# przemo199/ray-tracer-challenge-rs

Measured on AMD Instinct MI355X. Metric: Mray/s (primary+secondary) and ms/frame at 1920x1080, higher is better.
Workload: dtype f32; 1 GPU; three_sphere_scene@1920x1080,depth=5,f32; scene=three_sphere_scene, width=1920, height=1080, max_depth=5, out=real, parallelism=framesx1, rays_per_frame=4147200, stream=side, mode=frames

## Files before the change

### include/rtc_scene.h

```cpp
#ifndef RTC_SCENE_H
#define RTC_SCENE_H

#include "rtc.h"

#ifdef __cplusplus
extern "C" {
#endif

typedef struct rt_scene rt_scene;

typedef struct rt_scene_view {
    const rt_shape_desc* shapes;
    uint32_t n_shapes;
    const rt_material_desc* materials;
    uint32_t n_materials;
    const rt_pattern_desc* patterns;
    uint32_t n_patterns;
    const rt_light_desc* lights;
    uint32_t n_lights;
    rt_camera_desc camera;
    uint32_t duplicate_shapes;
} rt_scene_view;

int rt_scene_load_yaml(const char* path, rt_scene** out);
// ... 9 lines not shown
    const uint32_t* triangles;
    uint32_t n_triangles;
    uint32_t ignored_lines;
} rt_mesh_view;

int rt_mesh_load_obj(const char* path, rt_mesh** out);
int rt_mesh_load_obj_text(const char* text, rt_mesh** out);
int rt_mesh_view_get(const rt_mesh* mesh, rt_mesh_view* view);
void rt_mesh_free(rt_mesh* mesh);

int rt_mesh_triangles(const rt_mesh* mesh, const double* transform, int bake, int32_t material, rt_shape_desc* out);

#define RT_OBJ_NORMALS 1u
#define RT_NO_NORMAL 0xFFFFFFFFu
int rt_mesh_load_obj_ex(const char* path, const char* text, uint32_t flags, rt_mesh** out);

typedef struct rt_mesh_normals_view {
    const double* normals;
    uint32_t n_normals;
    uint32_t n_smooth;
    const uint32_t* triangle_normals;
} rt_mesh_normals_view;
int rt_mesh_normals_get(const rt_mesh* mesh, rt_mesh_normals_view* view);

int rt_mesh_smooth_normals(const rt_mesh* mesh, const double* transform, int bake, rt_smooth_desc* out,
                           uint32_t list, uint32_t* n_out);

#define RT_OBJ_TEXCOORDS 4u
#define RT_NO_TEXCOORD 0xFFFFFFFFu
typedef struct rt_mesh_texcoords_view {
    const double* texcoords;
    uint32_t n_texcoords;
    uint32_t n_textured;
    const uint32_t* triangle_texcoords;
} rt_mesh_texcoords_view;
int rt_mesh_texcoords_get(const rt_mesh* mesh, rt_mesh_texcoords_view* view);
int rt_mesh_uvs(const rt_mesh* mesh, rt_uv_desc* out, uint32_t list, uint32_t* n_out);

int rt_camera_make(uint32_t width, uint32_t height, double field_of_view,
                   const double from[3], const double to[3], const double up[3],
                   rt_camera_desc* out);

int rt_camera_resize(rt_camera_desc* camera, uint32_t width, uint32_t height);

int rt_camera_set_transform(rt_camera_desc* camera, const double transform[16]);

int rt_camera_bound_rect(const rt_camera_desc* camera, const float bound[4], uint32_t rect[4]);

int rt_camera_shadow_rect(const rt_camera_desc* camera, const float plane[4], const float light[3],
                          const float bound[4], uint32_t rect[4]);

int rt_camera_shadow_near(const rt_camera_desc* camera, const float plane[4], const float light[3], uint32_t span[4]);

int rt_matrix_inverse(const double m[16], double out[16]);

int rt_image_write(const char* path, const uint8_t* rgb, uint32_t width, uint32_t height);

enum {
    RT_IMAGE_AUTO = 0,
    RT_IMAGE_PNG = 1,
    RT_IMAGE_PPM = 2,
    RT_IMAGE_PPM_BINARY = 3
};
int rt_image_write_format(const char* path, const uint8_t* rgb, uint32_t width, uint32_t height, int format);

int rt_canvas_quantize(const double* rgb, uint64_t n_channels, uint8_t* out);

#ifdef __cplusplus
}
#endif

#endif
```

### ray-tracer-challenge-rs_amd/csrc/primary_rect.hpp

```cpp
#pragma once

#include <cmath>
#include <cstdint>

#include "rtc_internal.hpp"

namespace rtc {

enum ConicExtent { kConicFull, kConicOff, kConicRect };
struct ConicForm {
    double ad[3][3];
};
inline bool conic_form(const double m[3][3], const double oc[3], double R, ConicForm& f) {
    double g[3][3] = {}, q[3] = {}, oo = 0.0;
    for (int i = 0; i < 3; ++i)
        for (int j = 0; j < 3; ++j)
            for (int k = 0; k < 3; ++k) g[i][j] += m[k][i] * m[k][j];
    for (int i = 0; i < 3; ++i) oo += oc[i] * oc[i];
    for (int i = 0; i < 3; ++i)
        for (int k = 0; k < 3; ++k) q[i] += m[k][i] * oc[k];
    const double k = oo - R * R;
    if (!(k > 1e-6 * oo) || !std::isfinite(k)) return false;
    double c[3][3];
    for (int i = 0; i < 3; ++i)
// ... 175 lines not shown
        qa += S * S * f1 * f1, qb += S * S * f0 * f1, qc += S * S * f0 * f0;
        const double disc = qb * qb - qa * qc;
        if (!std::isfinite(disc) || !(disc > 0.0) || qa == 0.0) return false;
        const double root = std::sqrt(disc);
        const double u1 = (-qb - root) / qa, u2 = (-qb + root) / qa;
        if (qa < 0.0) {
            lo = u2, hi = u1;
            return f0 + f1 * 0.5 * (lo + hi) > 0.0;
        }
        if (f1 > 0.0) lo = u2, hi = HUGE_VAL;
        else if (f1 < 0.0) lo = -HUGE_VAL, hi = u1;
        else return false;
        return true;
    };
    auto axis = [&](bool rows, uint32_t n_pix, uint32_t n_other, uint32_t& lo, uint32_t& hi) {
        double lo_a, hi_a, lo_b, hi_b;
        const double e0 = -1.0, e1 = (double)n_other;
        if (rows ? !line_span(e0, 0.0, 0.0, 1.0, lo_a, hi_a) || !line_span(e1, 0.0, 0.0, 1.0, lo_b, hi_b)
                 : !line_span(0.0, e0, 1.0, 0.0, lo_a, hi_a) || !line_span(0.0, e1, 1.0, 0.0, lo_b, hi_b))
            return;
        const double a = std::fmax(std::fmax(lo_a, lo_b), -1.0), b = std::fmin(std::fmin(hi_a, hi_b), (double)n_pix);
        if (!(a <= b)) return;
        const double ai = std::ceil(a), bi = std::floor(b);
        if (!(ai <= bi)) return;
        if (rows ? !near_at(e0, ai) || !near_at(e1, ai) || !near_at(e0, bi) || !near_at(e1, bi)
                 : !near_at(ai, e0) || !near_at(ai, e1) || !near_at(bi, e0) || !near_at(bi, e1))
            return;
        if (ai + 1.0 > bi - 1.0) return;
        lo = (uint32_t)(ai + 1.0);
        hi = (uint32_t)(bi - 1.0);
    };
    axis(false, width, height, span[0], span[2]);
    axis(true, height, width, span[1], span[3]);
}

inline bool shadow_self_clear(const CameraRec<float>& cam, const float n[3], float h, const float light[3]) {
    double nn = 0.0, no = 0.0, nl = 0.0, omax = 0.0, lmax = 0.0;
    for (int i = 0; i < 3; ++i) {
        nn += (double)n[i] * n[i];
        no += (double)n[i] * cam.origin[i];
        nl += (double)n[i] * light[i];
        omax = std::fmax(omax, std::fabs((double)cam.origin[i]));
        lmax = std::fmax(lmax, std::fabs((double)light[i]));
    }
    nn = std::sqrt(nn);
    if (!(nn > 0.0) || !std::isfinite(nn)) return false;
    const double ye = (no - (double)h) / nn, yl = (nl - (double)h) / nn;
    const double scale = 1.0 + omax + lmax + std::fabs((double)h) / nn;
    if (!std::isfinite(ye) || !std::isfinite(yl) || !(ye * yl > 0.0)) return false;
    if (!(std::fabs(ye) > 1e-3 * scale) || !(std::fabs(yl) > 1e-3 * scale)) return false;
    const double over_max = 3e-6 * (1.0 + omax + std::fabs(ye) * nn / 8e-8);
    return over_max <= 1e3 * std::fabs(yl);
}
}
```

### ray-tracer-challenge-rs_amd/csrc/rtc_host.cpp

```cpp
#include <hip/hip_runtime.h>

#include <algorithm>
#include <array>
#include <chrono>
#include <cmath>
#include <cstdlib>
#include <cstring>
#include <limits>
#include <memory>
#include <string>
#include <vector>

#include "../../include/rtc.h"
#include "flop_model.hpp"
#include "host_math.hpp"
#include "debug_knobs.hpp"
#include "launch_terms.hpp"
#include "primary_rect.hpp"
#include "rtc_context.hpp"
#include "rtc_internal.hpp"
#include "shape_identity.hpp"
#include "tri_tree.hpp"
#include "instances.hpp"

// ... 854 lines not shown
        P.spill_blocks = (uint32_t)(ctx->d_spill.capacity() / per_block);
    }
    P.persistent = ls.sched;
    P.flags = flags;
    P.world_lds = ls.world_lds;
    const bool dynamic = ls.pool;
    if (dynamic) {
        const size_t set = (size_t)kTileQueues * kQueueStride;
        P.tile_counter = ctx->d_tile_counter.get() + (ctx->head_set ? set : 0);
        P.next_tile_counter = ctx->d_tile_counter.get() + (ctx->head_set ? 0 : set);
        if (ls.pool && ctx->knobs.tile_order && cam) {
            if ((rc = plan_tile_order<R>(ctx, lens ? ctx->order_lens : ss ? ctx->order_ss : ctx->order, P, cam, depth,
                                         ls.grid, stream, q.lens)))
                return rc;
        }
    }
    if (flags & RT_FLAG_STAMPS) {
        if ((rc = ctx->d_stamps.reserve((size_t)2 * ls.grid))) return rc;
        P.stamps = ctx->d_stamps.get();
        ctx->stamp_count = ls.grid;
        if (ls.pool) {
            const size_t items = (size_t)P.n_tiles << kMaxSplitLog2;
            if ((rc = ctx->d_item_log.reserve(1 + 3 * items))) return rc;
            RT_HIP(hipMemsetAsync(ctx->d_item_log.get(), 0, sizeof(uint64_t), stream));
            P.item_log = ctx->d_item_log.get();
        }
    }
    uint32_t kinds = 0;
    for (int k = 0; k < kNumKinds; ++k)
        if (w.scene.kind_begin[k + 1] > w.scene.kind_begin[k]) kinds |= 1u << k;
    const bool sp = sizeof(R) == 4 && ls.pool && ctx->knobs.kind_variants && (kinds & ~kKindsSp) == 0 && !dup && !ss &&
                    ctx->kernel_build == KernelBuild::plain;
    if (flags & RT_FLAG_FAIL_LAUNCH) return set_error(RT_ERR_HIP, "launch refused (RT_FLAG_FAIL_LAUNCH)");
    if constexpr (sizeof(R) == 4) {
        const size_t ns = ctx->jit.shapes.size();
        const bool small_direct = jf && !ls.pool && cam && !ss && ns <= (size_t)kPrimaryRectSlots &&
                                  (int)ns == w.scene.kind_begin[kNumKinds];
        if (small_direct) launch_terms(ctx->jit.shapes.data(), w.scene.kind_begin, (int)ns, P.cam.origin, P.terms);
        if (small_direct && P.width <= kCullCols * kCullCellW && P.height <= kCullRows * kCullCellH) {
            const uint32_t nc = (P.width + kCullCellW - 1) / kCullCellW, nr = (P.height + kCullCellH - 1) / kCullCellH;
            uint32_t flip_cols[kCullCols + 1] = {}, flip_rows[kCullRows + 1] = {};
            auto outside = [&](const uint32_t r[4], uint32_t b) {
                const bool none = r[0] > r[2] || r[1] > r[3];
                const uint32_t c0 = none ? nc : r[0] / kCullCellW, c1 = none ? nc : r[2] / kCullCellW + 1;
                const uint32_t r0 = none ? nr : r[1] / kCullCellH, r1 = none ? nr : r[3] / kCullCellH + 1;
                flip_cols[0] ^= b, flip_cols[c0] ^= b, flip_cols[c1] ^= b;
                flip_rows[0] ^= b, flip_rows[r0] ^= b, flip_rows[r1] ^= b;
            };
            for (size_t s = 0; s < ns; ++s) {
                uint32_t r[4];
                primary_rect(P.cam, P.width, P.height, ctx->jit.shapes[s].bound, r);
                outside(r, 1u << s);
            }
            const ShadowLayout lay(w.scene.kind_begin, (int)ctx->jit.lights.size());
            if (lay.fits() &&(int)ctx->jit.lights.size() == w.scene.n_lights) {
                for (int p = lay.plane0; p < lay.plane0 + lay.planes; ++p) {
                    const ShapeRec<float>& pl = ctx->jit.shapes[p];
                    const float n[3] = {pl.inv[4], pl.inv[5], pl.inv[6]}, h = -pl.inv[7];
                    uint32_t near[4] = {0, 0, P.width - 1, P.height - 1};
                    for (int l = 0; l < lay.lights; ++l) {
                        const float* lp = ctx->jit.lights[l].position;
                        uint32_t sp[4];
                        shadow_near(P.cam, P.width, P.height, n, h, lp, sp);
                        for (int a = 0; a < 2; ++a) {
                            near[a] = sp[a] > near[a] ? sp[a] : near[a];
                            near[a + 2] = sp[a + 2] < near[a + 2] ? sp[a + 2] : near[a + 2];
                        }
                        for (size_t c = 0; c < ns; ++c) {
                            const int bit = lay.pair_bit(l, p, (int)c);
                            if (bit < 0) continue;
                            if ((int)c == p) {
                                if (shadow_self_clear(P.cam, n, h, lp)) flip_cols[0] ^= 1u << bit;
                                continue;
                            }
                            uint32_t r[4];
                            shadow_rect(P.cam, P.width, P.height, n, h, lp, ctx->jit.shapes[c].bound, r);
                            outside(r, 1u << bit);
                        }
                    }
                    auto blocks = [](uint32_t lo, uint32_t hi, uint32_t cell, uint32_t pixels, uint32_t& b0, uint32_t& b1) {
                        b0 = b1 = 0;
                        if (lo > hi) return;
                        b0 = (lo + cell - 1) / cell;
                        b1 = hi + 1 >= pixels ? (pixels + cell - 1) / cell : (hi + 1) / cell;
                        if (b1 < b0) b1 = b0;
                    };
                    const uint32_t nb = 1u << lay.near_bit(p);
                    uint32_t b0, b1;
                    blocks(near[0], near[2], kCullCellW, P.width, b0, b1);
                    flip_cols[b0] ^= nb, flip_cols[b1] ^= nb;
                    blocks(near[1], near[3], kCullCellH, P.height, b0, b1);
                    flip_rows[b0] ^= nb, flip_rows[b1] ^= nb;
                }
            }
            uint32_t acc = 0;
            for (uint32_t i = 0; i < nc; ++i) P.cull_cols[i] = acc ^= flip_cols[i];
            acc = 0;
            for (uint32_t j = 0; j < nr; ++j) P.cull_rows[j] = acc ^= flip_rows[j];
        }
    }
    if (jf) {
        const ShapeRec<R>* sh = P.scene.shapes;
        const MaterialRec<R>* mt = P.scene.materials;
        const PatternRec<R>* pt = P.scene.patterns;
        const LightRec<R>* lt = P.scene.lights;
        void* args[] = {&P, &sh, &mt, &pt, &lt, &lens_params};
// ... 1715 lines not shown
```

### ray-tracer-challenge-rs_amd/csrc/rtc_kernels.hip

```cpp
#ifndef RTC_INSTANCES
#define RTC_INSTANCES 0
#endif
#ifndef RTC_AREA_LIGHTS
#define RTC_AREA_LIGHTS 0
#endif
#ifndef RTC_TEXTURES
#define RTC_TEXTURES 0
#endif
#if defined(RTC_VARIANT) && !RTC_INSTANCES
#define RTC_POOL_ONLY 1
#endif
#ifndef __HIPCC_RTC__
#include <hip/hip_runtime.h>

#include <cstdint>
#endif

#include "rtc_internal.hpp"

namespace rtc {
#ifdef RTC_VARIANT
namespace RTC_VARIANT {
#endif

// ... 743 lines not shown
            const int32_t e = P.inst_pos[inst[k].pos_begin + (hw - inst[k].world_base)];
            const bool plain = inst[k].expanded != 0;
            h.slot = plain ? (int)((uint32_t)e & 0xFFFFFFu) : e;
            h.kind = plain ? (int)((uint32_t)e >> 24) : (RT_SHAPE_TRIANGLE | ((k + 1) << 8));
            return h;
        }
#endif
        if (hw != __INT_MAX__) {
            const uint32_t ws = (uint32_t)sc.lworld_slot[hw];
            h.slot = (int)(ws & 0xFFFFFFu);
            h.kind = (int)(ws >> 24);
        }
        return h;
    }
};

#ifndef RTC_CUBE_EXIT_PATH
#define RTC_CUBE_EXIT_PATH 1
#endif
template <typename R>
__device__ inline bool jit_cube_holds_light(const ShapeRec<R>& s) {
#if defined(RTC_JIT) && RTC_CUBE_EXIT_PATH
    if constexpr (sizeof(R) == 4) {
        bool any = false;
        for (int i = 0; i < jit::kNumLights; ++i) {
            const V3<R> p = xform_point(s.inv, V3<R>{jit::kLights[i].position[0], jit::kLights[i].position[1],
                                                     jit::kLights[i].position[2]});
            constexpr R kIn = (R)(1 - 1e-4);
            any |= Real<R>::fabs(p.x) < kIn && Real<R>::fabs(p.y) < kIn && Real<R>::fabs(p.z) < kIn;
        }
        return any;
    }
#endif
    (void)s;
    return false;
}

template <typename R>
__device__ inline bool skips_on(const DevScene<R>& sc) {
#ifdef RTC_NO_SKIPS
    (void)sc;
    return false;
#else
#ifdef RTC_JIT
    if constexpr (sizeof(R) == 4) return true;
#endif
    return !sc.no_skips;
#endif
}

#ifndef RTC_PRIMARY_RECTS
#define RTC_PRIMARY_RECTS 1
#endif
struct NoBlock {
    static constexpr bool kOn = false;
    __device__ bool misses(int) const { return false; }
    __device__ float plane_height(int) const { return 0.0f; }
    __device__ float origin_max() const { return 0.0f; }
};
#ifndef RTC_LAUNCH_TERMS
#define RTC_LAUNCH_TERMS 1
#endif
#ifdef RTC_JIT
constexpr int kJitPlane0 = jit::kBegin[RT_SHAPE_PLANE];
constexpr int kJitPlanes = jit::kBegin[RT_SHAPE_PLANE + 1] - kJitPlane0;
#else
constexpr int kJitPlane0 = 0, kJitPlanes = 0;
#endif
struct PixelBlock {
    static constexpr bool kOn = true;
    uint32_t miss;
    __device__ inline bool misses(int slot) const { return (miss >> slot) & 1u; }
    static constexpr int kHead = kJitPlanes <= kPrimaryRectSlots ? (1 + kJitPlanes + 3) / 4 * 4 : 4;
    float head[kHead];
    __device__ inline float plane_height(int plane) const { return head[1 + plane]; }
    __device__ inline float origin_max() const { return head[0]; }
};

template <typename R, typename B = NoBlock>
__device__ inline Hit<R> closest_hit(const DevScene<R>& sc, V3<R> o, V3<R> d, B blk = B{}) {
    Nearest<R> best;
#if defined(RTC_JIT) && !defined(RTC_NO_SKIPS) && RTC_PRIMARY_RECTS
    constexpr bool kRects = B::kOn && sizeof(R) == 4 && jit::kBegin[kNumKinds] <= kPrimaryRectSlots;
    constexpr bool kLazy = kRects && jit::kNumClusters == 0;
#else
    constexpr bool kRects = false, kLazy = false;
#endif
#if defined(RTC_JIT) && RTC_LAUNCH_TERMS
    constexpr bool kTerms = B::kOn && sizeof(R) == 4 && jit::kBegin[kNumKinds] <= kPrimaryRectSlots;
#else
    constexpr bool kTerms = false;
#endif
    R dd0 = (R)0, rdd0 = (R)0;
    V3<R> rd0 = {(R)0, (R)0, (R)0};
    if constexpr (!kLazy) {
        dd0 = dot(d, d);
        rdd0 = recip(dd0);
        rd0 = recip3(d);
    }
    for_all_culled<R, true>(sc, o, d, dd0, [&]<int K>(const ShapeRec<R>& s, int slot) {
        if constexpr (kTerms) jit_fence_dir(d, slot);
        else jit_fence(o, d, slot);
        if constexpr (kRects && K != RT_SHAPE_PLANE)
            if (blk.misses(slot)) return;
        const R dd = kLazy ? dot(d, d) : dd0;
        if (!wave_may_hit<R, K>(s, o, d, dd)) return;
        const int w = kJitRecords && sizeof(R) == 4 ? (s.world_index << 8) | slot : s.world_index;
        if (world_sphere<R, K>(s)) {
            const R rdd = kLazy ? recip(dd) : rdd0;
            sphere_world<R, true>(s, o, d, dd, rdd, [&](R t, bool v) { best.offer(t, v, w); });
            return;
        }
        if (world_cube<R, K>(s)) {
            const V3<R> rd = kLazy ? recip3(d) : rd0;
            cube_world<R, true>(s, o, d, rd, [&](R t, bool v) { best.offer(t, v, w); });
            return;
        }
        V3<R> lo = {(R)0, (R)0, (R)0};
        if constexpr (kTerms && K == RT_SHAPE_PLANE) lo.y = blk.plane_height(slot - kJitPlane0);
        else lo = xform_point(s.inv, o);
        const V3<R> ld = xform_vector(s.inv, d);
        if (K == RT_SHAPE_PLANE && skips_on(sc)) {
            if (!wave_any(!(lo.y * ld.y > (R)0))) return;
        }
        if constexpr (K == RT_SHAPE_CUBE && sizeof(R) == 4) {
            if (jit_cube_holds_light(s) && skips_on(sc) &&
                !wave_any(!(Real<R>::fabs(lo.x) < (R)1 && Real<R>::fabs(lo.y) < (R)1 && Real<R>::fabs(lo.z) < (R)1))) {
                using T = Real<R>;
                auto hi = [](auto org, auto dir) {
                    const bool steep = T::fabs(dir) >= T::kEps;
                    const R r = sel(steep, __builtin_amdgcn_rcpf(dir), T::kMax);
                    return sel(r > (R)0, (R)1 - org, (R)-1 - org) * r;
                };
                const R tmax = T::fmin(T::fmin(T::fmin(T::kMax, hi(lo.x, ld.x)), hi(lo.y, ld.y)), hi(lo.z, ld.z));
                best.offer(tmax, tmax > (R)0, w);
                return;
            }
        }
        entries<R, K, true>(s, lo, ld, [&](R t, bool v) { best.offer(t, v, w); });
    });
    return best.hit(sc);
}

template <typename R>
struct Blocker {
    static constexpr bool kKeys = sizeof(R) == 4 && RTC_VALU_KEYS;
    bool hit = false;
    uint32_t tmin = 0x7F800000u;
    __device__ inline void offer(R t, bool v, R dist) {
        if constexpr (kKeys) {
            const uint32_t b = __float_as_uint((v ? t : -1.0f) + 0.0f);
            tmin = b < tmin ? b : tmin;
        } else {
            hit |= v & (t >= (R)0) & (t < dist);
        }
    }
// ... 2170 lines not shown
```

### ray-tracer-challenge-rs_amd/csrc/scene_loader.cpp

```cpp
#include <cerrno>
#include <cstdlib>
#include <cstring>
#include <fstream>
#include <map>
#include <memory>
#include <sstream>
#include <stdexcept>
#include <string>
#include <vector>

#include "../../include/rtc_scene.h"
#include "host_math.hpp"
#include "primary_rect.hpp"
#include "rtc_internal.hpp"
#include "shape_identity.hpp"

namespace rtc {
namespace {

using hm::M4;

struct Node {
    enum Kind { Bad, Null, Bool, Int, Real, Str, Seq, Map } kind = Bad;
    bool b = false;
    int64_t i = 0;
    std::string s;
    std::vector<Node> seq;
    std::vector<std::pair<std::string, Node>> map;

    const Node& operator[](const std::string& key) const {
        static const Node bad;
        if (kind != Map) return bad;
        const Node* hit = &bad;
        for (const auto& kv : map)
            if (kv.first == key) hit = &kv.second;
        return *hit;
    }
    bool is_bad() const { return kind == Bad; }
};

[[noreturn]] void fail(const std::string& msg) { throw std::runtime_error(msg); }

bool rust_parse_f64(const std::string& v, double& out) {
    std::string t = v;
    size_t p = 0;
    if (p < t.size() && (t[p] == '+' || t[p] == '-')) ++p;
    std::string rest = t.substr(p);
    std::string low;
    for (char c : rest) low += (char)std::tolower((unsigned char)c);
    if (low == "inf" || low == "infinity" || low == "nan") {
        double r = (low == "nan") ? NAN : INFINITY;
        out = (t[0] == '-') ? -r : r;
        return true;
    }
    size_t q = p, digits = 0;
    while (q < t.size() && std::isdigit((unsigned char)t[q])) ++q, ++digits;
    if (q < t.size() && t[q] == '.') {
        ++q;
        while (q < t.size() && std::isdigit((unsigned char)t[q])) ++q, ++digits;
    }
    if (digits == 0) return false;
    if (q < t.size() && (t[q] == 'e' || t[q] == 'E')) {
        ++q;
        if (q < t.size() && (t[q] == '+' || t[q] == '-')) ++q;
        size_t e = 0;
// ... 704 lines not shown
}

int rt_camera_set_transform(rt_camera_desc* cam, const double t[16]) {
    if (!cam || !t) return rtc::set_error(RT_ERR_INVALID, "rt_camera_set_transform: null argument");
    rtc::hm::M4 a;
    for (int r = 0; r < 4; ++r)
        for (int c = 0; c < 4; ++c) a.m[r][c] = t[4 * r + c];
    const rtc::hm::M4 inv = rtc::hm::inverse(a);
    for (int r = 0; r < 4; ++r)
        for (int c = 0; c < 4; ++c) cam->inverse[4 * r + c] = inv.m[r][c];
    const double o[3] = {0, 0, 0};
    rtc::hm::mul_point(inv, o, cam->origin);
    return RT_OK;
}

int rt_camera_bound_rect(const rt_camera_desc* cam, const float bound[4], uint32_t rect[4]) {
    if (!cam || !bound || !rect) return rtc::set_error(RT_ERR_INVALID, "rt_camera_bound_rect: null argument");
    if (cam->width == 0 || cam->height == 0) return rtc::set_error(RT_ERR_INVALID, "rt_camera_bound_rect: empty canvas");
    rtc::CameraRec<float> c;
    for (int q = 0; q < 12; ++q) c.inv[q] = (float)cam->inverse[q];
    for (int q = 0; q < 3; ++q) c.origin[q] = (float)cam->origin[q];
    c.half_width = (float)cam->half_width;
    c.half_height = (float)cam->half_height;
    c.pixel_size = (float)cam->pixel_size;
    rtc::primary_rect(c, cam->width, cam->height, bound, rect);
    return RT_OK;
}

static rtc::CameraRec<float> launch_camera(const rt_camera_desc* cam) {
    rtc::CameraRec<float> c;
    for (int q = 0; q < 12; ++q) c.inv[q] = (float)cam->inverse[q];
    for (int q = 0; q < 3; ++q) c.origin[q] = (float)cam->origin[q];
    c.half_width = (float)cam->half_width;
    c.half_height = (float)cam->half_height;
    c.pixel_size = (float)cam->pixel_size;
    return c;
}

int rt_camera_shadow_rect(const rt_camera_desc* cam, const float plane[4], const float light[3], const float bound[4],
                          uint32_t rect[4]) {
    if (!cam || !plane || !light || !bound || !rect) return rtc::set_error(RT_ERR_INVALID, "rt_camera_shadow_rect: null argument");
    if (cam->width == 0 || cam->height == 0) return rtc::set_error(RT_ERR_INVALID, "rt_camera_shadow_rect: empty canvas");
    rtc::shadow_rect(launch_camera(cam), cam->width, cam->height, plane, plane[3], light, bound, rect);
    return RT_OK;
}

int rt_camera_shadow_near(const rt_camera_desc* cam, const float plane[4], const float light[3], uint32_t span[4]) {
    if (!cam || !plane || !light || !span) return rtc::set_error(RT_ERR_INVALID, "rt_camera_shadow_near: null argument");
    if (cam->width == 0 || cam->height == 0) return rtc::set_error(RT_ERR_INVALID, "rt_camera_shadow_near: empty canvas");
    rtc::shadow_near(launch_camera(cam), cam->width, cam->height, plane, plane[3], light, span);
    return RT_OK;
}

int rt_matrix_inverse(const double m[16], double out[16]) {
    if (!m || !out) return rtc::set_error(RT_ERR_INVALID, "rt_matrix_inverse: null argument");
    rtc::hm::M4 a;
    for (int r = 0; r < 4; ++r)
        for (int c = 0; c < 4; ++c) a.m[r][c] = m[4 * r + c];
    rtc::hm::M4 inv = rtc::hm::inverse(a);
    for (int r = 0; r < 4; ++r)
        for (int c = 0; c < 4; ++c) out[4 * r + c] = inv.m[r][c];
    return RT_OK;
}

}
```

### ray-tracer-challenge-rs_amd/rtc_amd/__init__.py

```python
from __future__ import annotations

import ctypes as C
import os
from dataclasses import dataclass

import numpy as np

__all__ = [
    "RenderError", "lib_path", "abi_version", "device_count", "matrix_inverse", "camera_make",
    "camera_resize", "camera_set_transform", "camera_bound_rect", "load_scene", "load_scene_text", "SceneTables", "Context", "shard_rows",
    "load_obj", "Mesh", "SmoothDesc", "RT_SMOOTH_SHAPES", "RT_OBJ_NORMALS", "RT_NO_NORMAL",
    "AreaLightDesc", "RT_LIGHT_MAX_STEPS", "RT_JITTER_NONE", "RT_JITTER_HASHED", "area_light_sample",
    "LensDesc", "Lens", "lens_ray",
    "UVDesc", "TextureDesc", "RT_OBJ_TEXCOORDS", "RT_NO_TEXCOORD", "TEXTURE_FILTERS", "read_image",
    "RT_DEFAULT_MAX_DEPTH", "RT_TILE_H", "RT_TILE_W",
]

RT_ABI_VERSION = 3
RT_TILE_W = 64
RT_TILE_H = 4
RT_DEFAULT_MAX_DEPTH = 6
RT_MAX_SUPPORTED_DEPTH = 16
RT_MAX_SAMPLE_GRID = 4

RT_OK = 0
RT_ERR_INVALID, RT_ERR_HIP, RT_ERR_NO_DEVICE, RT_ERR_NO_SCENE = -1, -2, -3, -4
RT_ERR_OOM, RT_ERR_POOL, RT_ERR_IO, RT_ERR_COMM = -5, -6, -7, -8
STATUS = {0: "RT_OK", -1: "RT_ERR_INVALID", -2: "RT_ERR_HIP", -3: "RT_ERR_NO_DEVICE", -4: "RT_ERR_NO_SCENE",
          -5: "RT_ERR_OOM", -6: "RT_ERR_POOL", -7: "RT_ERR_IO", -8: "RT_ERR_COMM"}
RT_UNIQUE_ID_BYTES = 128
RT_IPC_HANDLE_BYTES = 64
RT_GATHER_RCCL, RT_GATHER_PEER = 0, 1
RT_SMOOTH_SHAPES = 0xFFFFFFFF
RT_OBJ_NORMALS = 1
RT_NO_NORMAL = 0xFFFFFFFF
RT_OBJ_TEXCOORDS = 4
RT_NO_TEXCOORD = 0xFFFFFFFF
TEXTURE_FILTERS = {"nearest": 0, "bilinear": 1}
RT_LIGHT_MAX_STEPS = 16
RT_JITTER_NONE, RT_JITTER_HASHED = 0, 1

SHAPE_KINDS = {"sphere": 0, "plane": 1, "cube": 2, "cylinder": 3, "cone": 4, "triangle": 5}
PATTERN_KINDS = {"stripe": 0, "gradient": 1, "ring": 2, "checker": 3, "complex": 4, "test": 5, "image": 6}
PRECISIONS = {"f32": 0, "f64": 1}
RT_FLAG_NO_COUNTERS, RT_FLAG_NO_SHADE, RT_FLAG_NO_TRACE, RT_FLAG_STAMPS, RT_FLAG_FAIL_LAUNCH = 1, 2, 4, 8, 16
RT_FLAG_GENERATIONS = 32
RT_FLAG_NO_SKIPS = 64
RT_JIT_OFF, RT_JIT_SYNC, RT_JIT_AUTO, RT_JIT_EAGER = 0, 1, 2, 3
OUT_FORMATS = {"real": 0, "u8": 1}


class RenderError(RuntimeError):
    def __init__(self, code: int, message: str):
        super().__init__(f"{STATUS.get(code, code)}: {message}")
        self.code = code


class ShapeDesc(C.Structure):
    _fields_ = [("kind", C.c_int32), ("material", C.c_int32), ("inverse", C.c_double * 16),
                ("minimum", C.c_double), ("maximum", C.c_double), ("closed", C.c_int32),
                ("reserved", C.c_int32), ("vertex_1", C.c_double * 3), ("edge_1", C.c_double * 3),
                ("edge_2", C.c_double * 3), ("normal", C.c_double * 3)]

# ... 199 lines not shown
        "rt_scene_upload_instanced": (C.c_int, [C.c_void_p, P(ShapeDesc), C.c_uint32, P(MeshDesc), C.c_uint32,
                                                P(InstanceDesc), C.c_uint32, P(MaterialDesc), C.c_uint32,
                                                P(PatternDesc), C.c_uint32, P(LightDesc), C.c_uint32]),
        "rt_instances_expand": (C.c_int, [P(ShapeDesc), C.c_uint32, P(MeshDesc), C.c_uint32, P(InstanceDesc),
                                          C.c_uint32, P(ShapeDesc)]),
        "rt_scene_instance_info": (C.c_int, [C.c_void_p, P(InstanceInfo)]),
        "rt_scene_upload_smooth": (C.c_int, [C.c_void_p, P(ShapeDesc), C.c_uint32, P(MeshDesc), C.c_uint32,
                                             P(InstanceDesc), C.c_uint32, P(SmoothDesc), C.c_uint32,
                                             P(MaterialDesc), C.c_uint32, P(PatternDesc), C.c_uint32, P(LightDesc),
                                             C.c_uint32]),
        "rt_smooth_expand": (C.c_int, [P(ShapeDesc), C.c_uint32, P(MeshDesc), C.c_uint32, P(InstanceDesc), C.c_uint32,
                                       P(SmoothDesc), C.c_uint32, P(SmoothDesc), P(C.c_uint32)]),
        "rt_scene_smooth_info": (C.c_int, [C.c_void_p, P(SmoothInfo)]),
        "rt_mesh_load_obj_ex": (C.c_int, [C.c_char_p, C.c_char_p, C.c_uint32, P(C.c_void_p)]),
        "rt_mesh_normals_get": (C.c_int, [C.c_void_p, P(MeshNormalsView)]),
        "rt_mesh_smooth_normals": (C.c_int, [C.c_void_p, P(C.c_double), C.c_int, P(SmoothDesc), C.c_uint32,
                                             P(C.c_uint32)]),
        "rt_scene_upload_textured": (C.c_int, [C.c_void_p, P(ShapeDesc), C.c_uint32, P(MeshDesc), C.c_uint32,
                                               P(InstanceDesc), C.c_uint32, P(SmoothDesc), C.c_uint32, P(UVDesc),
                                               C.c_uint32, P(TextureDesc), C.c_uint32, P(MaterialDesc), C.c_uint32,
                                               P(PatternDesc), C.c_uint32, P(LightDesc), C.c_uint32]),
        "rt_uv_expand": (C.c_int, [P(ShapeDesc), C.c_uint32, P(MeshDesc), C.c_uint32, P(InstanceDesc), C.c_uint32,
                                   P(UVDesc), C.c_uint32, P(UVDesc), P(C.c_uint32)]),
        "rt_scene_texture_info": (C.c_int, [C.c_void_p, P(TextureInfo)]),
        "rt_scene_upload_lit": (C.c_int, [C.c_void_p, P(ShapeDesc), C.c_uint32, P(MeshDesc), C.c_uint32,
                                          P(InstanceDesc), C.c_uint32, P(SmoothDesc), C.c_uint32, P(UVDesc),
                                          C.c_uint32, P(TextureDesc), C.c_uint32, P(MaterialDesc), C.c_uint32,
                                          P(PatternDesc), C.c_uint32, P(LightDesc), C.c_uint32, P(AreaLightDesc),
                                          C.c_uint32]),
        "rt_lights_expand": (C.c_int, [P(LightDesc), C.c_uint32, P(AreaLightDesc), C.c_uint32, P(LightDesc),
                                       P(C.c_uint32)]),
        "rt_render_lens": (C.c_int, [C.c_void_p, P(CameraDesc), P(RenderOptions), C.c_uint32, P(LensDesc), C.c_void_p,
                                     P(Stats)]),
        "rt_render_lens_device": (C.c_int, [C.c_void_p, P(CameraDesc), P(RenderOptions), C.c_uint32, P(LensDesc),
                                            C.c_void_p, C.c_void_p]),
        "rt_lens_ray": (C.c_int, [P(CameraDesc), C.c_uint32, P(LensDesc), C.c_uint32, C.c_uint32, C.c_uint32, C.c_uint32,
                                  P(C.c_double)]),
        "rt_area_light_sample": (C.c_int, [P(AreaLightDesc), C.c_uint32, C.c_uint32, C.c_uint32, C.c_uint32,
                                           P(C.c_double)]),
        "rt_scene_light_info": (C.c_int, [C.c_void_p, P(LightInfo)]),
        "rt_mesh_texcoords_get": (C.c_int, [C.c_void_p, P(MeshTexcoordsView)]),
        "rt_mesh_uvs": (C.c_int, [C.c_void_p, P(UVDesc), C.c_uint32, P(C.c_uint32)]),
        "rt_image_read": (C.c_int, [C.c_char_p, P(P(C.c_uint8)), P(C.c_uint32), P(C.c_uint32)]),
        "rt_image_free": (None, [P(C.c_uint8)]),
        "rt_image_write": (C.c_int, [C.c_char_p, C.c_void_p, C.c_uint32, C.c_uint32]),
        "rt_image_write_format": (C.c_int, [C.c_char_p, C.c_void_p, C.c_uint32, C.c_uint32, C.c_int]),
        "rt_canvas_quantize": (C.c_int, [P(C.c_double), C.c_uint64, P(C.c_uint8)]),
        "rt_camera_make": (C.c_int, [C.c_uint32, C.c_uint32, C.c_double, P(C.c_double), P(C.c_double),
                                     P(C.c_double), P(CameraDesc)]),
        "rt_camera_resize": (C.c_int, [P(CameraDesc), C.c_uint32, C.c_uint32]),
        "rt_camera_bound_rect": (C.c_int, [P(CameraDesc), P(C.c_float), P(C.c_uint32)]),
        "rt_camera_shadow_rect": (C.c_int, [P(CameraDesc), P(C.c_float), P(C.c_float), P(C.c_float), P(C.c_uint32)]),
        "rt_camera_shadow_near": (C.c_int, [P(CameraDesc), P(C.c_float), P(C.c_float), P(C.c_uint32)]),
        "rt_matrix_inverse": (C.c_int, [P(C.c_double), P(C.c_double)]),
        "rt_camera_set_transform": (C.c_int, [P(CameraDesc), P(C.c_double)]),
        "rt_shard_row_map": (C.c_int, [C.c_uint32, C.c_uint32, P(C.c_uint32), P(C.c_uint32)]),
        "rt_context_create_multi": (C.c_int, [P(C.c_int), C.c_int, P(C.c_void_p)]),
        "rt_comm_unique_id": (C.c_int, [P(C.c_uint8)]),
        "rt_context_create_rank": (C.c_int, [C.c_int, C.c_int, C.c_int, P(C.c_uint8), P(C.c_void_p)]),
        "rt_context_group": (C.c_int, [C.c_void_p, P(C.c_int), P(C.c_int), P(C.c_int)]),
        "rt_context_set_jit": (C.c_int, [C.c_void_p, C.c_int]),
        "rt_context_set_frames_in_flight": (C.c_int, [C.c_void_p, C.c_uint32]),
        "rt_jit_status": (C.c_int, [C.c_void_p, P(C.c_int), P(C.c_double), C.c_char_p, C.c_size_t]),
        "rt_jit_wait": (C.c_int, [C.c_void_p, C.c_double, P(C.c_int)]),
        "rt_canvas_create": (C.c_int, [C.c_void_p, C.c_uint64, C.c_uint32, P(C.c_void_p), P(C.c_uint8)]),
        "rt_canvas_open": (C.c_int, [C.c_void_p, P(C.c_uint8), C.c_uint64, C.c_uint32, P(C.c_void_p)]),
        "rt_canvas_close": (C.c_int, [C.c_void_p, C.c_void_p]),
        "rt_render_to_canvas": (C.c_int, [C.c_void_p, P(CameraDesc), P(RenderOptions), C.c_void_p, C.c_uint64,
                                          C.c_double, C.c_void_p]),
        "rt_canvas_wait": (C.c_int, [C.c_void_p, C.c_void_p, C.c_uint64, C.c_double, C.c_void_p]),
        "rt_canvas_release": (C.c_int, [C.c_void_p, C.c_void_p, C.c_uint64, C.c_void_p]),
        "rt_canvas_read": (C.c_int, [C.c_void_p, C.c_void_p, C.c_void_p, C.c_uint64]),
        "rt_context_set_gather": (C.c_int, [C.c_void_p, C.c_int]),
        "rt_debug_intersect": (C.c_int, [C.c_void_p, C.c_uint32, P(C.c_double), C.c_uint64, C.c_uint32, C.c_uint32,
                                         P(C.c_double)]),
        "rt_debug_normal": (C.c_int, [C.c_void_p, C.c_uint32, P(C.c_double), C.c_uint64, C.c_uint32, C.c_uint32,
                                      P(C.c_double)]),
    }
    for name, (res, args) in sig.items():
        fn = getattr(lib, name)
        fn.restype = res
        fn.argtypes = args
    if lib.rt_abi_version() != RT_ABI_VERSION:
        raise ImportError(f"rtc_amd: {path} has ABI {lib.rt_abi_version()}, this module expects {RT_ABI_VERSION}")
    return lib


_lib = _load()

EXPORTED_SYMBOLS = (
    "rt_abi_version", "rt_last_error", "rt_device_count", "rt_context_create", "rt_context_destroy",
    "rt_scene_upload", "rt_shard_rows", "rt_render", "rt_render_device", "rt_color_at", "rt_read_counters",
    "rt_trace_rays", "rt_trace_rays_device", "rt_render_supersampled", "rt_render_supersampled_device",
    "rt_read_generation_counts",
    "rt_debug_stamps", "rt_debug_tile_costs", "rt_debug_item_log", "rt_debug_intersect", "rt_debug_normal", "rt_camera_set_transform",
    "rt_shard_row_map", "rt_context_create_multi", "rt_comm_unique_id", "rt_context_create_rank", "rt_context_group",
    "rt_context_set_jit", "rt_context_set_frames_in_flight", "rt_jit_status", "rt_jit_wait", "rt_canvas_create", "rt_canvas_open", "rt_canvas_close",
    "rt_render_to_canvas", "rt_canvas_wait", "rt_canvas_release", "rt_canvas_read", "rt_context_set_gather",
    "rt_assemble_shards", "rt_scene_load_yaml", "rt_scene_load_yaml_text", "rt_scene_view_get", "rt_scene_free",
    "rt_camera_make", "rt_camera_resize", "rt_camera_bound_rect", "rt_camera_shadow_rect", "rt_camera_shadow_near",
    "rt_matrix_inverse", "rt_image_write", "rt_image_write_format",
    "rt_canvas_quantize",
    "rt_mesh_load_obj", "rt_mesh_load_obj_text", "rt_mesh_view_get", "rt_mesh_free", "rt_mesh_triangles",
    "rt_scene_tree_info",
    "rt_scene_upload_instanced", "rt_instances_expand", "rt_scene_instance_info",
    "rt_scene_upload_smooth", "rt_smooth_expand", "rt_scene_smooth_info",
    "rt_mesh_load_obj_ex", "rt_mesh_normals_get", "rt_mesh_smooth_normals",
    "rt_scene_upload_textured", "rt_uv_expand", "rt_scene_texture_info", "rt_mesh_texcoords_get", "rt_mesh_uvs",
    "rt_image_read", "rt_image_free",
    "rt_scene_upload_lit", "rt_lights_expand", "rt_area_light_sample", "rt_scene_light_info",
    "rt_render_lens", "rt_render_lens_device", "rt_lens_ray",
)


def _check(rc: int) -> None:
    if rc != RT_OK:
        raise RenderError(rc, _lib.rt_last_error().decode(errors="replace"))


def abi_version() -> int:
    return _lib.rt_abi_version()


def device_count() -> int:
    n = C.c_int(0)
    _check(_lib.rt_device_count(C.byref(n)))
    return n.value


def matrix_inverse(m) -> np.ndarray:
    a = (C.c_double * 16)(*np.asarray(m, dtype=np.float64).reshape(16))
    out = (C.c_double * 16)()
    _check(_lib.rt_matrix_inverse(a, out))
    return np.array(out[:], dtype=np.float64).reshape(4, 4)


def camera_make(width: int, height: int, fov: float, frm, to, up) -> CameraDesc:
    cam = CameraDesc()
    v = lambda x: (C.c_double * 3)(*[float(t) for t in x])
    _check(_lib.rt_camera_make(width, height, float(fov), v(frm), v(to), v(up), C.byref(cam)))
    return cam


def camera_set_transform(cam: CameraDesc, transform) -> CameraDesc:
    c = cam.copy()
    t = (C.c_double * 16)(*np.asarray(transform, dtype=np.float64).reshape(16))
    _check(_lib.rt_camera_set_transform(C.byref(c), t))
    return c


def camera_resize(cam: CameraDesc, width: int, height: int) -> CameraDesc:
    c = cam.copy()
    _check(_lib.rt_camera_resize(C.byref(c), width, height))
    return c


def camera_bound_rect(cam: CameraDesc, bound) -> tuple:
    b = (C.c_float * 4)(*np.asarray(bound, dtype=np.float32).reshape(4))
    r = (C.c_uint32 * 4)()
    _check(_lib.rt_camera_bound_rect(C.byref(cam), b, r))
    return tuple(r[:])


def _f32s(values, n):
    return (C.c_float * n)(*np.asarray(values, dtype=np.float32).reshape(n))


def camera_shadow_rect(cam: CameraDesc, plane, light, bound) -> tuple:
    r = (C.c_uint32 * 4)()
    _check(_lib.rt_camera_shadow_rect(C.byref(cam), _f32s(plane, 4), _f32s(light, 3), _f32s(bound, 4), r))
    return tuple(r[:])


def camera_shadow_near(cam: CameraDesc, plane, light) -> tuple:
    r = (C.c_uint32 * 4)()
    _check(_lib.rt_camera_shadow_near(C.byref(cam), _f32s(plane, 4), _f32s(light, 3), r))
    return tuple(r[:])


IMAGE_FORMATS = {"auto": 0, "png": 1, "ppm": 2, "ppm-binary": 3}


def write_image(path, image: np.ndarray, fmt: str = "auto") -> None:
    img = np.ascontiguousarray(image)
    if img.dtype != np.uint8 or img.ndim != 3 or img.shape[2] != 3:
        raise ValueError("write_image takes a uint8 array of shape (H, W, 3)")
    _check(_lib.rt_image_write_format(os.fsencode(path), img.ctypes.data if img.size else None, img.shape[1],
                                      img.shape[0], IMAGE_FORMATS[fmt]))


def read_image(path) -> np.ndarray:
    rgb, w, h = C.POINTER(C.c_uint8)(), C.c_uint32(0), C.c_uint32(0)
    _check(_lib.rt_image_read(os.fsencode(path), C.byref(rgb), C.byref(w), C.byref(h)))
    try:
        return np.ctypeslib.as_array(rgb, (h.value, w.value, 3)).copy()
    finally:
        _lib.rt_image_free(rgb)


def Lens(aperture: float, focal_distance: float, jitter: bool = False, seed: int = 0) -> "LensDesc":
    return LensDesc(float(aperture), float(focal_distance), RT_JITTER_HASHED if jitter else RT_JITTER_NONE,
                    int(seed) & 0xFFFFFFFF)


def lens_ray(camera: "CameraDesc", grid: int, lens: "LensDesc", x: int, y: int, i: int, j: int) -> np.ndarray:
    ray = (C.c_double * 6)()
    _check(_lib.rt_lens_ray(C.byref(camera), grid, C.byref(lens), x, y, i, j, ray))
    return np.array(ray[:], dtype=np.float64)


def area_light_sample(desc: "AreaLightDesc", area_index: int, ray_id: int, remaining: int, k: int) -> np.ndarray:
    pos = (C.c_double * 3)()
    _check(_lib.rt_area_light_sample(C.byref(desc), area_index, ray_id, remaining, k, pos))
    return np.array(pos[:], dtype=np.float64)


def canvas_quantize(image: np.ndarray) -> np.ndarray:
    src = np.ascontiguousarray(image, dtype=np.float64)
    out = np.zeros(src.shape, dtype=np.uint8)
    _check(_lib.rt_canvas_quantize(src.ctypes.data_as(C.POINTER(C.c_double)), src.size,
                                   out.ctypes.data_as(C.POINTER(C.c_uint8))))
    return out


def shard_rows(height: int, shard_count: int) -> int:
    r = C.c_uint32(0)
    _check(_lib.rt_shard_rows(height, shard_count, C.byref(r)))
    return r.value

# ... 594 lines not shown
```

Baseline: 471,200 Mray/s.

## Cull primary rays against planes using conservative screen-space visibility rectangles

Computes, on the host, a conservative pixel rectangle per plane where that plane can be the nearest primary hit, by clipping the screen polygon against the plane's horizon line and against regions where other planes are closer. The rectangles feed the existing tile-cull bitmask, and the kernel now lets planes skip intersection tests in tiles outside their rectangle. This targets wasted plane intersection work for primary rays. It adds host-side geometry with error bounds, and a too-tight bound could drop visible hits.

```diff
diff --git a/include/rtc_scene.h b/include/rtc_scene.h
--- a/include/rtc_scene.h
+++ b/include/rtc_scene.h
@@ -85,6 +85,9 @@
 
 int rt_camera_shadow_near(const rt_camera_desc* camera, const float plane[4], const float light[3], uint32_t span[4]);
 
+int rt_camera_plane_rect(const rt_camera_desc* camera, const float* planes, uint32_t n_planes, uint32_t q,
+                         uint32_t rect[4]);
+
 int rt_matrix_inverse(const double m[16], double out[16]);
 
 int rt_image_write(const char* path, const uint8_t* rgb, uint32_t width, uint32_t height);
diff --git a/ray-tracer-challenge-rs_amd/csrc/primary_rect.hpp b/ray-tracer-challenge-rs_amd/csrc/primary_rect.hpp
--- a/ray-tracer-challenge-rs_amd/csrc/primary_rect.hpp
+++ b/ray-tracer-challenge-rs_amd/csrc/primary_rect.hpp
@@ -251,4 +251,141 @@
     const double over_max = 3e-6 * (1.0 + omax + std::fabs(ye) * nn / 8e-8);
     return over_max <= 1e3 * std::fabs(yl);
 }
-}
+
+struct PlaneView {
+    bool ok = false;
+    double m[3][3];
+    double hw, hh, ps;
+    double eps, dmax;
+    uint32_t width, height;
+};
+inline void plane_view(const CameraRec<float>& cam, uint32_t width, uint32_t height, PlaneView& v) {
+    v.ok = false;
+    v.width = width, v.height = height;
+    v.hw = cam.half_width, v.hh = cam.half_height, v.ps = cam.pixel_size;
+    auto& m = v.m;
+    for (int i = 0; i < 3; ++i)
+        for (int j = 0; j < 3; ++j) m[i][j] = cam.inv[4 * i + j];
+    if (!(v.ps > 0.0) || !std::isfinite(v.hw) || !std::isfinite(v.hh) || !std::isfinite(v.ps)) return;
+    const double det = m[0][0] * (m[1][1] * m[2][2] - m[1][2] * m[2][1]) - m[0][1] * (m[1][0] * m[2][2] - m[1][2] * m[2][0]) +
+                       m[0][2] * (m[1][0] * m[2][1] - m[1][1] * m[2][0]);
+    double adj2 = 0.0, s2 = 0.0;
+    for (int i = 0; i < 3; ++i) {
+        const int i1 = (i + 1) % 3, i2 = (i + 2) % 3;
+        for (int j = 0; j < 3; ++j) {
+            const int j1 = (j + 1) % 3, j2 = (j + 2) % 3;
+            const double c = m[i1][j1] * m[i2][j2] - m[i1][j2] * m[i2][j1];
+            adj2 += c * c;
+        }
+        const double s = std::fabs(m[i][0]) * (std::fabs(v.hw) + v.ps) + std::fabs(m[i][1]) * (std::fabs(v.hh) + v.ps) +
+                         std::fabs(m[i][2]);
+        s2 += s * s;
+    }
+    if (!std::isfinite(det) || !std::isfinite(adj2) || !std::isfinite(s2) || !(std::fabs(det) > 1e-12 * std::sqrt(adj2) * std::sqrt(s2)))
+        return;
+    const double dmin = std::fabs(det) / std::sqrt(adj2);
+    v.dmax = 0.0;
+    for (int c = 0; c < 4; ++c) {
+        const double wx = v.hw - ((c & 1 ? (double)width : -1.0) + 0.5) * v.ps, wy = v.hh - ((c & 2 ? (double)height : -1.0) + 0.5) * v.ps;
+        double dd = 0.0;
+        for (int i = 0; i < 3; ++i) {
+            const double d = m[i][0] * wx + m[i][1] * wy - m[i][2];
+            dd += d * d;
+        }
+        v.dmax = std::fmax(v.dmax, std::sqrt(dd));
+    }
+    constexpr double eta = 1.0 / 16777216.0;
+    v.eps = 2.0 * eta * (6.0 * std::sqrt(s2) / dmin + 5.0);
+    v.ok = std::isfinite(v.eps) && std::isfinite(v.dmax) && v.eps < 1e-3 && v.dmax > 0.0;
+}
+struct PlaneLine {
+    bool ok = false;
+    double a, b, c;
+    double side;
+    double gap;
+};
+inline void plane_line(const PlaneView& v, const float row[4], float h, PlaneLine& l) {
+    l.ok = false;
+    if (!v.ok) return;
+    const double n[3] = {row[0], row[1], row[2]}, s = -(double)h;
+    const double nn = std::sqrt(n[0] * n[0] + n[1] * n[1] + n[2] * n[2]), sa = std::fabs(s);
+    if (!std::isfinite(nn) || !std::isfinite(sa) || !(nn > 1e-15) || !(nn < 1e15) || !(sa > 1e-15 * nn) || !(sa < 1e15 * nn)) return;
+    double nm[3];
+    for (int j = 0; j < 3; ++j) nm[j] = (n[0] * v.m[0][j] + n[1] * v.m[1][j] + n[2] * v.m[2][j]) / s;
+    l.a = -nm[0] * v.ps;
+    l.b = -nm[1] * v.ps;
+    l.c = nm[0] * (v.hw - 0.5 * v.ps) + nm[1] * (v.hh - 0.5 * v.ps) - nm[2];
+    const double g = nn / sa;
+    l.side = (100.0 * v.eps + 1e-6 / nn) * g * v.dmax;
+    l.gap = 100.1 * v.eps * g * v.dmax;
+    l.ok = std::fabs(l.a) < 1e100 && std::fabs(l.b) < 1e100 && std::fabs(l.c) < 1e100 && l.side < 1e100 && l.gap < 1e100;
+}
+struct PlanePoly {
+    static constexpr int kMax = 16;
+    int n = 0;
+    double x[kMax], y[kMax];
+    void clip(double a, double b, double c) {
+        double ox[kMax], oy[kMax], f[kMax];
+        for (int i = 0; i < n; ++i) f[i] = a * x[i] + b * y[i] + c;
+        int k = 0;
+        for (int i = 0; i < n && k + 2 <= kMax; ++i) {
+            const int j = i + 1 == n ? 0 : i + 1;
+            if (f[i] >= 0.0) ox[k] = x[i], oy[k] = y[i], ++k;
+            if ((f[i] >= 0.0) != (f[j] >= 0.0)) {
+                const double t = f[i] / (f[i] - f[j]);
+                ox[k] = x[i] + t * (x[j] - x[i]), oy[k] = y[i] + t * (y[j] - y[i]), ++k;
+            }
+        }
+        n = k;
+        for (int i = 0; i < k; ++i) x[i] = ox[i], y[i] = oy[i];
+    }
+    void extend(double box[4]) const {
+        for (int i = 0; i < n; ++i) {
+            box[0] = std::fmin(box[0], x[i]), box[1] = std::fmin(box[1], y[i]);
+            box[2] = std::fmax(box[2], x[i]), box[3] = std::fmax(box[3], y[i]);
+        }
+    }
+};
+inline void plane_rect(const PlaneView& v, const PlaneLine* lines, int n, int q, uint32_t rect[4]) {
+    rect_full(v.width, v.height, rect);
+    if (!v.ok || q < 0 || q >= n || n > kPrimaryRectSlots || !lines[q].ok) return;
+    const PlaneLine& lq = lines[q];
+    constexpr double kappa = 400.0 / 16777216.0;
+    PlanePoly aq;
+    aq.n = 4;
+    aq.x[0] = aq.x[3] = -1.0, aq.x[1] = aq.x[2] = (double)v.width;
+    aq.y[0] = aq.y[1] = -1.0, aq.y[2] = aq.y[3] = (double)v.height;
+    aq.clip(lq.a, lq.b, lq.c + lq.side);
+    double box[4] = {-HUGE_VAL, -HUGE_VAL, HUGE_VAL, HUGE_VAL};
+    for (int p = 0; p < n && aq.n; ++p) {
+        if (p == q || !lines[p].ok) continue;
+        const PlaneLine& lp = lines[p];
+        PlanePoly behind = aq;
+        behind.clip(-lp.a, -lp.b, lp.side - lp.c);
+        const double rhs = lp.gap + lq.gap + 1.001 * lq.side;
+        const double la = lq.a * (1.0 + kappa) - lp.a * (1.0 - kappa), lb = lq.b * (1.0 + kappa) - lp.b * (1.0 - kappa),
+                     lc = rhs + lq.c * (1.0 + kappa) - lp.c * (1.0 - kappa);
+        if (behind.n == 0) {
+            aq.clip(la, lb, lc);
+            continue;
+        }
+        PlanePoly level = aq;
+        level.clip(la, lb, lc);
+        double bp[4] = {HUGE_VAL, HUGE_VAL, -HUGE_VAL, -HUGE_VAL};
+        behind.extend(bp);
+        level.extend(bp);
+        box[0] = std::fmax(box[0], bp[0]), box[1] = std::fmax(box[1], bp[1]);
+        box[2] = std::fmin(box[2], bp[2]), box[3] = std::fmin(box[3], bp[3]);
+    }
+    double bq[4] = {HUGE_VAL, HUGE_VAL, -HUGE_VAL, -HUGE_VAL};
+    aq.extend(bq);
+    box[0] = std::fmax(box[0], bq[0]), box[1] = std::fmax(box[1], bq[1]);
+    box[2] = std::fmin(box[2], bq[2]), box[3] = std::fmin(box[3], bq[3]);
+    if (!(box[0] == box[0]) || !(box[1] == box[1]) || !(box[2] == box[2]) || !(box[3] == box[3])) return;
+    const double x0 = std::floor(box[0]) - 1.0, y0 = std::floor(box[1]) - 1.0, x1 = std::ceil(box[2]) + 1.0, y1 = std::ceil(box[3]) + 1.0;
+    const double xm = (double)(v.width - 1), ym = (double)(v.height - 1);
+    if (!(x0 <= x1) || !(y0 <= y1) || x1 < 0.0 || y1 < 0.0 || x0 > xm || y0 > ym) return rect_empty(rect);
+    rect[0] = (uint32_t)(x0 < 0.0 ? 0.0 : x0), rect[1] = (uint32_t)(y0 < 0.0 ? 0.0 : y0);
+    rect[2] = (uint32_t)(x1 > xm ? xm : x1), rect[3] = (uint32_t)(y1 > ym ? ym : y1);
+}
+}
diff --git a/ray-tracer-challenge-rs_amd/csrc/rtc_host.cpp b/ray-tracer-challenge-rs_amd/csrc/rtc_host.cpp
--- a/ray-tracer-challenge-rs_amd/csrc/rtc_host.cpp
+++ b/ray-tracer-challenge-rs_amd/csrc/rtc_host.cpp
@@ -930,6 +930,18 @@
                 primary_rect(P.cam, P.width, P.height, ctx->jit.shapes[s].bound, r);
                 outside(r, 1u << s);
             }
+            const int p0 = w.scene.kind_begin[RT_SHAPE_PLANE], np = w.scene.kind_begin[RT_SHAPE_PLANE + 1] - p0;
+            if (np > 0) {
+                PlaneView pv;
+                PlaneLine pl[kPrimaryRectSlots];
+                plane_view(P.cam, P.width, P.height, pv);
+                for (int p = 0; p < np; ++p) plane_line(pv, ctx->jit.shapes[p0 + p].inv + 4, P.terms.head[1 + p], pl[p]);
+                for (int p = 0; p < np; ++p) {
+                    uint32_t r[4];
+                    plane_rect(pv, pl, np, p, r);
+                    outside(r, 1u << (p0 + p));
+                }
+            }
             const ShadowLayout lay(w.scene.kind_begin, (int)ctx->jit.lights.size());
             if (lay.fits() &&(int)ctx->jit.lights.size() == w.scene.n_lights) {
                 for (int p = lay.plane0; p < lay.plane0 + lay.planes; ++p) {
diff --git a/ray-tracer-challenge-rs_amd/csrc/rtc_kernels.hip b/ray-tracer-challenge-rs_amd/csrc/rtc_kernels.hip
--- a/ray-tracer-challenge-rs_amd/csrc/rtc_kernels.hip
+++ b/ray-tracer-challenge-rs_amd/csrc/rtc_kernels.hip
@@ -819,6 +819,9 @@
 #ifndef RTC_PRIMARY_RECTS
 #define RTC_PRIMARY_RECTS 1
 #endif
+#ifndef RTC_PLANE_RECTS
+#define RTC_PLANE_RECTS 1
+#endif
 struct NoBlock {
     static constexpr bool kOn = false;
     __device__ bool misses(int) const { return false; }
@@ -868,7 +871,7 @@
     for_all_culled<R, true>(sc, o, d, dd0, [&]<int K>(const ShapeRec<R>& s, int slot) {
         if constexpr (kTerms) jit_fence_dir(d, slot);
         else jit_fence(o, d, slot);
-        if constexpr (kRects && K != RT_SHAPE_PLANE)
+        if constexpr (kRects && (K != RT_SHAPE_PLANE || RTC_PLANE_RECTS))
             if (blk.misses(slot)) return;
         const R dd = kLazy ? dot(d, d) : dd0;
         if (!wave_may_hit<R, K>(s, o, d, dd)) return;
diff --git a/ray-tracer-challenge-rs_amd/csrc/scene_loader.cpp b/ray-tracer-challenge-rs_amd/csrc/scene_loader.cpp
--- a/ray-tracer-challenge-rs_amd/csrc/scene_loader.cpp
+++ b/ray-tracer-challenge-rs_amd/csrc/scene_loader.cpp
@@ -11,6 +11,7 @@
 
 #include "../../include/rtc_scene.h"
 #include "host_math.hpp"
+#include "launch_terms.hpp"
 #include "primary_rect.hpp"
 #include "rtc_internal.hpp"
 #include "shape_identity.hpp"
@@ -821,6 +822,24 @@
     return RT_OK;
 }
 
+int rt_camera_plane_rect(const rt_camera_desc* cam, const float* planes, uint32_t n_planes, uint32_t q, uint32_t rect[4]) {
+    if (!cam || !planes || !rect) return rtc::set_error(RT_ERR_INVALID, "rt_camera_plane_rect: null argument");
+    if (cam->width == 0 || cam->height == 0) return rtc::set_error(RT_ERR_INVALID, "rt_camera_plane_rect: empty canvas");
+    if (n_planes == 0 || n_planes > (uint32_t)rtc::kPrimaryRectSlots || q >= n_planes)
+        return rtc::set_error(RT_ERR_INVALID, "rt_camera_plane_rect: 1 to 8 planes, q one of them");
+    const rtc::CameraRec<float> c = launch_camera(cam);
+    rtc::PlaneView view;
+    rtc::PlaneLine lines[rtc::kPrimaryRectSlots];
+    rtc::plane_view(c, cam->width, cam->height, view);
+    for (uint32_t p = 0; p < n_planes; ++p) {
+        const float* m = planes + 4 * p;
+        const float h = rtc::launch_kfma(m[2], c.origin[2], rtc::launch_kfma(m[1], c.origin[1], rtc::launch_kfma(m[0], c.origin[0], m[3])));
+        rtc::plane_line(view, m, h, lines[p]);
+    }
+    rtc::plane_rect(view, lines, (int)n_planes, (int)q, rect);
+    return RT_OK;
+}
+
 int rt_matrix_inverse(const double m[16], double out[16]) {
     if (!m || !out) return rtc::set_error(RT_ERR_INVALID, "rt_matrix_inverse: null argument");
     rtc::hm::M4 a;
diff --git a/ray-tracer-challenge-rs_amd/rtc_amd/__init__.py b/ray-tracer-challenge-rs_amd/rtc_amd/__init__.py
--- a/ray-tracer-challenge-rs_amd/rtc_amd/__init__.py
+++ b/ray-tracer-challenge-rs_amd/rtc_amd/__init__.py
@@ -8,7 +8,7 @@
 
 __all__ = [
     "RenderError", "lib_path", "abi_version", "device_count", "matrix_inverse", "camera_make",
-    "camera_resize", "camera_set_transform", "camera_bound_rect", "load_scene", "load_scene_text", "SceneTables", "Context", "shard_rows",
+    "camera_resize", "camera_set_transform", "camera_bound_rect", "camera_plane_rect", "load_scene", "load_scene_text", "SceneTables", "Context", "shard_rows",
     "load_obj", "Mesh", "SmoothDesc", "RT_SMOOTH_SHAPES", "RT_OBJ_NORMALS", "RT_NO_NORMAL",
     "AreaLightDesc", "RT_LIGHT_MAX_STEPS", "RT_JITTER_NONE", "RT_JITTER_HASHED", "area_light_sample",
     "LensDesc", "Lens", "lens_ray",
@@ -314,6 +314,7 @@
         "rt_camera_bound_rect": (C.c_int, [P(CameraDesc), P(C.c_float), P(C.c_uint32)]),
         "rt_camera_shadow_rect": (C.c_int, [P(CameraDesc), P(C.c_float), P(C.c_float), P(C.c_float), P(C.c_uint32)]),
         "rt_camera_shadow_near": (C.c_int, [P(CameraDesc), P(C.c_float), P(C.c_float), P(C.c_uint32)]),
+        "rt_camera_plane_rect": (C.c_int, [P(CameraDesc), P(C.c_float), C.c_uint32, C.c_uint32, P(C.c_uint32)]),
         "rt_matrix_inverse": (C.c_int, [P(C.c_double), P(C.c_double)]),
         "rt_camera_set_transform": (C.c_int, [P(CameraDesc), P(C.c_double)]),
         "rt_shard_row_map": (C.c_int, [C.c_uint32, C.c_uint32, P(C.c_uint32), P(C.c_uint32)]),
@@ -361,7 +362,7 @@
     "rt_render_to_canvas", "rt_canvas_wait", "rt_canvas_release", "rt_canvas_read", "rt_context_set_gather",
     "rt_assemble_shards", "rt_scene_load_yaml", "rt_scene_load_yaml_text", "rt_scene_view_get", "rt_scene_free",
     "rt_camera_make", "rt_camera_resize", "rt_camera_bound_rect", "rt_camera_shadow_rect", "rt_camera_shadow_near",
-    "rt_matrix_inverse", "rt_image_write", "rt_image_write_format",
+    "rt_camera_plane_rect", "rt_matrix_inverse", "rt_image_write", "rt_image_write_format",
     "rt_canvas_quantize",
     "rt_mesh_load_obj", "rt_mesh_load_obj_text", "rt_mesh_view_get", "rt_mesh_free", "rt_mesh_triangles",
     "rt_scene_tree_info",
@@ -437,6 +438,13 @@
 def camera_shadow_near(cam: CameraDesc, plane, light) -> tuple:
     r = (C.c_uint32 * 4)()
     _check(_lib.rt_camera_shadow_near(C.byref(cam), _f32s(plane, 4), _f32s(light, 3), r))
+    return tuple(r[:])
+
+
+def camera_plane_rect(cam: CameraDesc, planes, q: int) -> tuple:
+    rows = np.ascontiguousarray(planes, dtype=np.float32).reshape(-1, 4)
+    r = (C.c_uint32 * 4)()
+    _check(_lib.rt_camera_plane_rect(C.byref(cam), _f32s(rows, rows.size), rows.shape[0], int(q), r))
     return tuple(r[:])
 
 
```

Result: faster. 503,200 Mray/s (median of 6 runs) (+6.8%).
